# isl-org/Open3D-PointNet2-Semantic3D

Hardware: AMD Instinct MI355X
Metric: points/sec through SA+FP stack (B=16,N=8192) (higher is better)
Workload: dtype f32

## Files before the change

### include/pn2_abi.h

```cpp
#ifndef PN2_ABI_H_
#define PN2_ABI_H_

#include <stddef.h>
#include <stdint.h>

#ifdef __cplusplus
extern "C" {
#endif

#define PN2_ABI_VERSION 2

#define PN2_OK 0
#define PN2_EINVAL (-1)
#define PN2_ENULL (-2)
#define PN2_ERANGE (-3)
#define PN2_EUNSUP (-4)

#define PN2_ARITH_STRICT 0
#define PN2_ARITH_FMA 1
#define PN2_ARITH_FMA_ALT 2

int pn2_abi_version(void);
const char *pn2_build_info(void);
const char *pn2_strerror(int code);
// ... 228 lines not shown
                                  const float *z, int nlayers, const int *widths, const float *const *w,
                                  const float *const *bias, float *y, int schedule, void *stream);

int pn2_set_sa_row_packing(int on);

int pn2_sa_mlp_fused_pre(int b, int n, int m, int nsample, const float *xyz, const float *new_xyz, const float *zf,
                         const int *idx, int nlayers, const int *widths, const float *const *w,
                         const float *const *bias, int pool, float *out, void *stream);

int pn2_fp_mlp_wide_pre(int b, int n, int m, int c1, const float *dist, const int *idx, const float *points1,
                        const float *z, int nlayers, const int *widths, const float *const *w,
                        const float *const *bias, float *y, void *stream);
int pn2_sa_mlp_wide_pre(int b, int n, int m, int nsample, const float *xyz, const float *new_xyz, const float *zf,
                        const int *idx, int nlayers, const int *widths, const float *const *w,
                        const float *const *bias, int pool, float *y, void *stream);

size_t pn2_ball_query_bin_bytes(int n);
int pn2_ball_query_bin(int b, int n, float radius, const float *xyz1, void *workspace, size_t workspace_bytes, void *stream);
int pn2_ball_query_bin_ld(int b, int n, float radius, const float *xyz1, int ld1, void *workspace, size_t workspace_bytes,
                          void *stream);
int pn2_query_ball_point_binned(int b, int n, int m, float radius, int nsample, const float *xyz1, const float *xyz2,
                                const void *bins, int *idx, int *pts_cnt, int arith_mode, void *stream);

int pn2_group_pool(long long rows, int k, int c, int mode, const float *x, const float *gxyz, float *out, void *stream);
int pn2_group_pool_grad(long long rows, int k, int c, int mode, const float *x, const float *gxyz, const float *dout,
                        float *dx, void *stream);

int pn2_bn_relu_forward_deferred(long long rows, int c, const float *y, const float *gamma, const float *beta,
                                 const float *bias, float eps, float decay, int stats_done, float *running_mean,
                                 float *running_var, void *workspace, size_t workspace_bytes, float *save_mean,
// ... 82 lines not shown
```

### open3d-pointnet2-semantic3d_amd/_lib.py

```python
import ctypes
import os
import sys

import torch

_HERE = os.path.dirname(os.path.abspath(__file__))
LIB_PATH = os.environ.get("PN2_HIP_LIBRARY") or os.path.join(_HERE, "libpn2_hip.so")

c_int, c_float, c_void_p = ctypes.c_int, ctypes.c_float, ctypes.c_void_p

SIGNATURES = {
    "pn2_farthest_point_sample": [c_int, c_int, c_int, c_void_p, c_void_p, c_void_p, c_int, c_void_p],
    "pn2_fps_gather": [c_int, c_int, c_int, c_void_p, c_void_p, c_void_p, c_void_p, c_int, c_void_p],
    "pn2_fps_nested": [c_int, c_int, c_int, c_void_p, c_void_p, c_void_p, c_void_p, c_void_p, c_void_p, c_int, c_void_p],
    "pn2_fps_nested_ld": [c_int, c_int, c_int, c_void_p, c_int, c_void_p, c_void_p, c_void_p, c_void_p, c_int, c_void_p],
    "pn2_coarse_geometry": [c_int, c_int, c_int, c_void_p, c_void_p, c_void_p, c_void_p, c_void_p, c_void_p, c_void_p, c_void_p,
                            c_void_p, c_void_p, c_void_p, c_void_p, c_int, c_int, c_void_p],
    "pn2_prob_sample": [c_int, c_int, c_int, c_void_p, c_void_p, c_void_p, c_void_p, c_void_p],
    "pn2_fps_large": [c_int, c_int, c_int, c_void_p, c_void_p, ctypes.c_size_t, c_void_p, c_void_p, c_int, c_void_p],
    "pn2_gather_point": [c_int, c_int, c_int, c_void_p, c_void_p, c_void_p, c_void_p],
    "pn2_gather_point_grad": [c_int, c_int, c_int, c_void_p, c_void_p, c_void_p, c_void_p],
    "pn2_query_ball_point": [c_int, c_int, c_int, c_float, c_int, c_void_p, c_void_p, c_void_p, c_void_p, c_int, c_void_p],
    "pn2_query_ball_point_ld": [c_int, c_int, c_int, c_float, c_int, c_void_p, c_int, c_void_p, c_void_p, c_void_p, c_int, c_void_p],
    "pn2_query_ball_point_kernel": [c_int, c_int, c_int, c_float, c_int, c_void_p, c_void_p, c_void_p, c_void_p, c_int, c_int,
# ... 109 lines not shown
                                c_void_p, c_void_p, c_void_p],
    "pn2_scene_sample": [c_int, c_int, c_int, c_void_p, c_void_p, c_void_p, c_void_p, c_void_p, c_void_p, ctypes.c_double,
                         ctypes.c_double, c_void_p, c_void_p, c_void_p, c_void_p, c_void_p, c_void_p, c_void_p],
    "pn2_fp_mlp_fused_pre": [c_int, c_int, c_int, c_int, c_void_p, c_void_p, c_void_p, c_void_p, c_int, c_void_p, c_void_p,
                             c_void_p, c_void_p, c_void_p],
    "pn2_fp_mlp_fused_pre_ld": [c_int, c_int, c_int, c_int, c_void_p, c_void_p, c_void_p, c_int, c_void_p, c_int, c_void_p, c_void_p,
                                c_void_p, c_void_p, c_void_p],
    "pn2_fp_mlp_fused_pre_schedule": [c_int, c_int, c_int, c_int, c_void_p, c_void_p, c_void_p, c_void_p, c_int, c_void_p,
                                      c_void_p, c_void_p, c_void_p, c_int, c_void_p],
    "pn2_sa_mlp_fused_pre": [c_int, c_int, c_int, c_int, c_void_p, c_void_p, c_void_p, c_void_p, c_int, c_void_p, c_void_p,
                             c_void_p, c_int, c_void_p, c_void_p],
    "pn2_fp_mlp_wide_pre": [c_int, c_int, c_int, c_int, c_void_p, c_void_p, c_void_p, c_void_p, c_int, c_void_p, c_void_p,
                            c_void_p, c_void_p, c_void_p],
    "pn2_sa_mlp_wide_pre": [c_int, c_int, c_int, c_int, c_void_p, c_void_p, c_void_p, c_void_p, c_int, c_void_p, c_void_p,
                            c_void_p, c_int, c_void_p, c_void_p],
    "pn2_ball_query_bin": [c_int, c_int, c_float, c_void_p, c_void_p, ctypes.c_size_t, c_void_p],
    "pn2_ball_query_bin_ld": [c_int, c_int, c_float, c_void_p, c_int, c_void_p, ctypes.c_size_t, c_void_p],
    "pn2_query_ball_point_binned": [c_int, c_int, c_int, c_float, c_int, c_void_p, c_void_p, c_void_p, c_void_p, c_void_p, c_int,
                                    c_void_p],
    "pn2_group_pool": [ctypes.c_longlong, c_int, c_int, c_int, c_void_p, c_void_p, c_void_p, c_void_p],
    "pn2_group_pool_grad": [ctypes.c_longlong, c_int, c_int, c_int, c_void_p, c_void_p, c_void_p, c_void_p, c_void_p],
    "pn2_voxel_downsample": [c_int, c_void_p, c_void_p, c_void_p, ctypes.c_double, c_void_p, c_void_p, c_void_p, c_void_p,
                             c_void_p, c_void_p, ctypes.c_size_t, c_void_p],
    "pn2_dataset_workspace_size": [c_int, c_int, c_void_p],
    "pn2_dataset_sample": [c_int, c_int, c_int, c_int, c_int, c_int, c_void_p, c_void_p, c_void_p, c_void_p, c_void_p, c_void_p,
                           c_void_p, c_int, ctypes.c_double, ctypes.c_double, ctypes.c_ulonglong, c_void_p, c_void_p, c_void_p,
                           c_void_p, c_int, c_void_p, c_void_p, ctypes.c_size_t, c_void_p, c_void_p, c_void_p, c_void_p,
                           c_void_p, c_void_p, c_void_p],
}
PN2_EUNSUP = -4
BN_WS_UNCLEARED, BN_WS_ZEROED, BN_WS_SUMMED, BN_WS_FOLDED = range(4)
_SIZE_QUERIES = {"pn2_fps_large_workspace_bytes": 2, "pn2_ball_query_bin_bytes": 1, "pn2_interpolate_label_workspace_bytes": 1,
                 "pn2_three_interpolate_grad_workspace_bytes": 3, "pn2_scatter_plan_bytes": 3,
                 "pn2_group_point_grad_workspace_bytes": 4, "pn2_voxel_downsample_workspace_bytes": 1, "pn2_bn_workspace_bytes": 1}
_TRACE_ARGS = {"pn2_sa_mlp_max_fused": (9, 10, None, ()), "pn2_sa_mlp_rows_fused": (9, 10, None, ()),
               "pn2_sa_mlp_max_fused_bf16": (9, 10, None, ()), "pn2_fp_mlp_fused": (9, 10, None, ()),
               "pn2_fp_mlp_wide_pre": (8, 9, None, ()), "pn2_sa_mlp_wide_pre": (8, 9, None, ()),
               "pn2_sa_mlp_fused_pre": (8, 9, None, ()), "pn2_fp_mlp_fused_pre": (8, 9, None, ()),
               "pn2_fp_mlp_fused_pre_schedule": (8, 9, None, ()), "pn2_mlp_chain": (3, 4, None, ()),
               "pn2_mlp_wide": (4, 5, None, ()), "pn2_fp_mlp_wide": (9, 10, None, ()), "pn2_sa_mlp_wide": (9, 10, None, ()),
               "pn2_fps_nested_ld": (None, None, "pn2_fps_nested", (3,)),
               "pn2_query_ball_point_ld": (None, None, "pn2_query_ball_point", (5,)),
               "pn2_three_nn_ld": (None, None, "pn2_three_nn", (3,)),
               "pn2_ball_query_bin_ld": (None, None, "pn2_ball_query_bin", (3,)),
               "pn2_sa_mlp_max_fused_ld": (11, 12, "pn2_sa_mlp_max_fused", (5, 6)),
               "pn2_fp_mlp_fused_pre_ld": (9, 10, "pn2_fp_mlp_fused_pre", (4,))}


class Pn2Error(RuntimeError):
    pass


def _load():
    import fcntl
    from . import build as _build
# ... 155 lines not shown
```

### open3d-pointnet2-semantic3d_amd/csrc/pn2_mlp_wide.hip

```cpp
#include "pn2_common.h"

namespace {

typedef float f32x4 __attribute__((ext_vector_type(4)));
typedef float f32x16 __attribute__((ext_vector_type(16)));

constexpr int kWideDepth = 4;

struct WideParams {
    int rows, cin, x_stride, nlayers, pool, relu_last;
    int w[3];
    const float* x;
    int n, m, c;
    const float* xyz;
    const float* new_xyz;
    const float* points;
    const int* idx;
    const float* dist;
    const float* points1;
    int c1, c2;
    const float* W[3];
    const float* bias[3];
    float* y;
    const float* zpre;
// ... 290 lines not shown
                    for (int t = 0; t < 4; ++t) acc[t][r] += z[t];
                }
            } else if constexpr (MODE == kWideGather) {
                const float* __restrict__ zb = p.zpre + (size_t)(tile / p.m) * p.n * N + cb + 4 * l31;
                const int* __restrict__ idx = p.idx + (size_t)tile * 32;
#pragma unroll
                for (int r = 0; r < 16; ++r) {
                    const int row = (r & 3) + 8 * (r >> 2) + 4 * half;
                    const f32x4 z = *reinterpret_cast<const f32x4*>(zb + (size_t)idx[row] * N);
#pragma unroll
                    for (int t = 0; t < 4; ++t) acc[t][r] += z[t];
                }
            }
        }
        if (ks == 0) {
            const f32x4 bv = *reinterpret_cast<const f32x4*>(p.bias[l] + cb + 4 * l31);
            const bool relu = !lastl || p.relu_last;
            if (!lastl) {
                float* __restrict__ out = smem + buf_off[(l + 1) & 1];
                const int so = p.sa[(l + 1) & 1];
#pragma unroll
                for (int r = 0; r < 16; ++r) {
                    const int row = (r & 3) + 8 * (r >> 2) + 4 * half;
                    f32x4 v = {acc[0][r] + bv[0], acc[1][r] + bv[1], acc[2][r] + bv[2], acc[3][r] + bv[3]};
                    v = {fmaxf(v[0], 0.f), fmaxf(v[1], 0.f), fmaxf(v[2], 0.f), fmaxf(v[3], 0.f)};
                    *reinterpret_cast<f32x4*>(out + row * so + cb + 4 * l31) = v;
                }
            } else if (p.pool == 32) {
                f32x4 v;
#pragma unroll
                for (int t = 0; t < 4; ++t) {
// ... 43 lines not shown
            if ((size_t)32 * p.sa[l & 1] < (size_t)2 * 64 * 64) alias_ok = false;
        }
        kin = p.w[l];
    }
    (void)kin;
    p.scratch_off = 32 * (p.sa[0] + p.sa[1]);
    p.scratch_alias = sliced && alias_ok;
    p.rowtab_off = p.scratch_off + (sliced && !alias_ok ? 2 * 64 * 64 : 0);
    const size_t lds = sizeof(float) * ((size_t)p.rowtab_off + (p.zpre && mode == kWideInterp ? 32 * 8 : 0));
    if (lds > kPn2CuLdsBytes) return PN2_EUNSUP;
    if (mode == kWideGather) return launch_mlp_wide_mode<kWideGather>(p, lds, st);
    if (mode == kWideInterp) return launch_mlp_wide_mode<kWideInterp>(p, lds, st);
    return launch_mlp_wide_mode<kWidePlain>(p, lds, st);
}

int check_layers(int nlayers, const int* widths, const float* const* w, const float* const* bias) {
    if (nlayers < 1 || nlayers > 3) return PN2_EUNSUP;
    if (!widths || !w || !bias) return PN2_ENULL;
    for (int l = 0; l < nlayers; ++l) {
        if (widths[l] != 128 && widths[l] != 256 && widths[l] != 512) return PN2_EUNSUP;
        if (!w[l] || !bias[l]) return PN2_ENULL;
        if ((((uintptr_t)w[l]) | ((uintptr_t)bias[l])) & 15) return PN2_EUNSUP;
    }
    return PN2_OK;
}

}

extern "C" int pn2_mlp_wide(int rows, int cin, int x_stride, const float* x, int nlayers, const int* widths,
                            const float* const* w, const float* const* bias, int relu_last, int pool, float* y, void* stream) {
    if (rows <= 0 || cin <= 0 || x_stride < cin) return PN2_EINVAL;
    if (!x || !y) return PN2_ENULL;
    int rc = check_layers(nlayers, widths, w, bias);
    if (rc != PN2_OK) return rc;
    if (pool != 0 && pool != 32) return PN2_EUNSUP;
    if (pool == 32 && rows % 32 != 0) return PN2_EINVAL;
    if (((uintptr_t)y) & 15) return PN2_EUNSUP;
    if ((long long)rows + 64 > 0x7fffffffLL) return PN2_ERANGE;
    WideParams p = {};
    p.rows = rows; p.cin = cin; p.x_stride = x_stride; p.nlayers = nlayers; p.pool = pool; p.relu_last = relu_last;
    p.x = x; p.y = y;
    for (int l = 0; l < nlayers; ++l) { p.w[l] = widths[l]; p.W[l] = w[l]; p.bias[l] = bias[l]; }
    return launch_mlp_wide(p, kWidePlain, static_cast<hipStream_t>(stream));
}

extern "C" int pn2_sa_mlp_wide(int b, int n, int m, int nsample, int c, const float* xyz, const float* new_xyz,
                               const float* points, const int* idx, int nlayers, const int* widths, const float* const* w,
                               const float* const* bias, int pool, float* y, void* stream) {
    if (b <= 0 || n <= 0 || m <= 0 || c <= 0) return PN2_EINVAL;
    if (!xyz || !new_xyz || !points || !idx || !y) return PN2_ENULL;
    if (nsample != 32 || c % 4 != 0 || (((uintptr_t)points | (uintptr_t)y) & 15)) return PN2_EUNSUP;
    int rc = check_layers(nlayers, widths, w, bias);
    if (rc != PN2_OK) return rc;
    if ((long long)b * m * 32 + 64 > 0x7fffffffLL) return PN2_ERANGE;
    WideParams p = {};
    p.rows = b * m * 32; p.cin = 3 + c; p.x_stride = 0; p.nlayers = nlayers; p.pool = pool ? 32 : 0; p.relu_last = 1;
    p.n = n; p.m = m; p.c = c; p.xyz = xyz; p.new_xyz = new_xyz; p.points = points; p.idx = idx; p.y = y;
    for (int l = 0; l < nlayers; ++l) { p.w[l] = widths[l]; p.W[l] = w[l]; p.bias[l] = bias[l]; }
// ... 4 lines not shown
                               const float* points2, int nlayers, const int* widths, const float* const* w,
                               const float* const* bias, float* y, void* stream) {
    if (b <= 0 || n <= 0 || m < 3 || c2 <= 0 || c1 < 0) return PN2_EINVAL;
    if (!dist || !idx || !points2 || !y || (c1 > 0 && !points1)) return PN2_ENULL;
    if (n % 32 != 0 || c2 % 4 != 0 || c1 % 4 != 0 || (((uintptr_t)points2 | (uintptr_t)points1 | (uintptr_t)y) & 15)) return PN2_EUNSUP;
    int rc = check_layers(nlayers, widths, w, bias);
    if (rc != PN2_OK) return rc;
    if ((long long)b * n + 64 > 0x7fffffffLL) return PN2_ERANGE;
    WideParams p = {};
    p.rows = b * n; p.cin = c2 + c1; p.nlayers = nlayers; p.pool = 0; p.relu_last = 1;
    p.n = n; p.m = m; p.c1 = c1; p.c2 = c2; p.dist = dist; p.idx = idx; p.points = points2; p.points1 = points1; p.y = y;
    for (int l = 0; l < nlayers; ++l) { p.w[l] = widths[l]; p.W[l] = w[l]; p.bias[l] = bias[l]; }
    return launch_mlp_wide(p, kWideInterp, static_cast<hipStream_t>(stream));
}

extern "C" int pn2_fp_mlp_wide_pre(int b, int n, int m, int c1, const float* dist, const int* idx, const float* points1,
                                   const float* z, int nlayers, const int* widths, const float* const* w,
                                   const float* const* bias, float* y, void* stream) {
    if (b <= 0 || n <= 0 || m < 3 || c1 <= 0) return PN2_EINVAL;
    if (!dist || !idx || !z || !y || !points1) return PN2_ENULL;
    if (n % 32 != 0 || c1 % 4 != 0 || (((uintptr_t)z | (uintptr_t)points1 | (uintptr_t)y) & 15)) return PN2_EUNSUP;
    int rc = check_layers(nlayers, widths, w, bias);
    if (rc != PN2_OK) return rc;
    if ((long long)b * n + 64 > 0x7fffffffLL) return PN2_ERANGE;
    WideParams p = {};
    p.rows = b * n; p.cin = c1; p.nlayers = nlayers; p.pool = 0; p.relu_last = 1;
    p.n = n; p.m = m; p.c1 = c1; p.c2 = 0; p.dist = dist; p.idx = idx; p.points = nullptr; p.points1 = points1; p.y = y; p.zpre = z;
    for (int l = 0; l < nlayers; ++l) { p.w[l] = widths[l]; p.W[l] = w[l]; p.bias[l] = bias[l]; }
    return launch_mlp_wide(p, kWideInterp, static_cast<hipStream_t>(stream));
}

extern "C" int pn2_sa_mlp_wide_pre(int b, int n, int m, int nsample, const float* xyz, const float* new_xyz, const float* zf,
                                   const int* idx, int nlayers, const int* widths, const float* const* w,
                                   const float* const* bias, int pool, float* y, void* stream) {
    if (b <= 0 || n <= 0 || m <= 0) return PN2_EINVAL;
    if (!xyz || !new_xyz || !zf || !idx || !y) return PN2_ENULL;
    if (nsample != 32 || (((uintptr_t)zf | (uintptr_t)y) & 15)) return PN2_EUNSUP;
    int rc = check_layers(nlayers, widths, w, bias);
    if (rc != PN2_OK) return rc;
    if ((long long)b * m * 32 + 64 > 0x7fffffffLL) return PN2_ERANGE;
    WideParams p = {};
    p.rows = b * m * 32; p.cin = 3; p.x_stride = 0; p.nlayers = nlayers; p.pool = pool ? 32 : 0; p.relu_last = 1;
    p.n = n; p.m = m; p.c = 4; p.xyz = xyz; p.new_xyz = new_xyz; p.points = zf; p.idx = idx; p.y = y; p.zpre = zf;
    for (int l = 0; l < nlayers; ++l) { p.w[l] = widths[l]; p.W[l] = w[l]; p.bias[l] = bias[l]; }
// ... 3 lines not shown
```

### open3d-pointnet2-semantic3d_amd/model.py

```python
import json

import torch

from .util import tf_util
from .util import pointnet_util as pu
from .util.pointnet_util import pointnet_fp_module, pointnet_sa_module
from .tf_ops.tf_interpolate import three_nn

SEMANTIC_HYPERPARAMS = {
    "num_point": 8192, "batch_size": 16, "use_color": 1,
    "optimizer": "adam", "momentum": 0.9, "learning_rate": 0.001, "decay_step": 200000, "learning_rate_decay_rate": 0.7,
    "bn_init_decay": 0.5, "bn_decay_decay_rate": 0.5, "bn_decay_clip": 0.99,
    "l1_radius": 0.5, "l1_nsample": 32, "l1_npoint": 1024,
    "l2_radius": 1.0, "l2_nsample": 32, "l2_npoint": 256,
    "l3_radius": 2.0, "l3_nsample": 32, "l3_npoint": 64,
    "l4_radius": 4.0, "l4_nsample": 32, "l4_npoint": 16,
}

SA_MLPS = ([32, 32, 64], [64, 64, 128], [128, 128, 256], [256, 256, 512])
FP_MLPS = ([256, 256], [256, 256], [256, 128], [128, 128, 128])


def load_hyperparams(path):
    with open(path) as f:
# ... 107 lines not shown
            xyzs[-1], feats[-1], npoint=hyperparams[k + "npoint"], radius=hyperparams[k + "radius"],
            nsample=hyperparams[k + "nsample"], mlp=list(SA_MLPS[li]), mlp2=None, group_all=False,
            is_training=is_training, bn_decay=bn_decay, scope="layer%d" % (li + 1), geometry=geo)
        if li == 0 and geometry is None:
            coarse = coarse_levels(new_xyz, hyperparams)
        xyzs.append(new_xyz)
        feats.append(new_points)

    fp_in = feats
    if cut_sa_fp and is_training:
        fp_in = [feats[0]] + [f.detach().requires_grad_(True) for f in feats[1:]]
        end_points["sa_features_cut"] = fp_in[1:]
    up = fp_in[4]
    for fi in range(4):
        lvl = 3 - fi
        up = pointnet_fp_module(xyzs[lvl], xyzs[lvl + 1], fp_in[lvl], up, list(FP_MLPS[fi]), is_training, bn_decay,
                                scope="fa_layer%d" % (fi + 1),
                                nn=(tuple(geometry["nn"][fi]) + (geometry.get("iplans", [None] * 4)[fi],) if geometry is not None
                                    else (tuple(coarse[2 - fi]["nn"]) + (None,) if (coarse is not None and fi < 3) else None)),
                                defer_last_bn=head_width if (fi == 3 and is_training) else 0)
    end_points["xyzs"] = xyzs
    end_points["sa_features"] = feats
    return up, end_points


def get_head(l0_points, is_training, num_class, bn_decay=None, end_points=None):
    net = tf_util.conv1d(l0_points, 128, 1, padding="VALID", bn=True, is_training=is_training, scope="fc1",
                         bn_decay=bn_decay)
    if end_points is not None:
        end_points["feats"] = net
    net = tf_util.dropout(net, keep_prob=0.5, is_training=is_training, scope="dp1")
    return tf_util.conv1d(net, num_class, 1, padding="VALID", activation_fn=None, scope="fc2", is_training=is_training)


def get_model(point_cloud, is_training, num_class, hyperparams, bn_decay=None, geometry=None, cut_sa_fp=False):
# ... 38 lines not shown
```

### open3d-pointnet2-semantic3d_amd/util/pointnet_util.py

```python

import torch

from . import tf_util
from .._lib import float_array, int_array, launch, lib, ptr, ptr_table, require_cuda, rows_in_place, u64_array
from ..tf_ops import tf_grouping
from ..tf_ops.tf_grouping import query_ball_point_multi, group_point, knn_point, query_ball_point
from ..tf_ops.tf_interpolate import three_interpolate, three_nn
from ..tf_ops.tf_sampling import (farthest_point_sample, farthest_point_sample_and_gather, farthest_point_sample_with_ties,
                                  gather_point, tag_fps_output)


def sample_and_group(npoint, radius, nsample, xyz, points, knn=False, use_xyz=True, geometry=None):
    plan = None
    if geometry is not None:
        new_xyz, idx = geometry[0], geometry[1]
        plan = geometry[2] if len(geometry) > 2 else None
    else:
        fps_idx, fps_tie, _ = farthest_point_sample_with_ties(npoint, xyz)
        new_xyz = tag_fps_output(gather_point(xyz, fps_idx), fps_tie)
        if knn:
            _, idx = knn_point(nsample, xyz, new_xyz)
        else:
            idx, pts_cnt = query_ball_point(radius, nsample, xyz, new_xyz)
    if USE_FUSED_TRAIN_FRONT and points is not None and use_xyz and points.dtype == torch.float32:
# ... 505 lines not shown
    return out


USE_FUSED_TRAIN_FRONT = True


USE_MLP_CHAIN = True


USE_MLP_WIDE = True
WIDE_MIN_ROWS = 4096


USE_FUSED_FP = True


def dense_mlp_inference(x2d, cin, mlp, scope_fmt, bn=True, fp_front=None):
    if x2d is None:
        dist, idx, points1, points2, pad_to = fp_front
        rows = dist.shape[0] * dist.shape[1]
        cw = -(-cin // pad_to) * pad_to
    else:
        rows, cw = x2d.shape
    folded = []
    c = cin
    for i, cout in enumerate(mlp):
        with tf_util.variable_scope(scope_fmt % i):
            pad_in = cw if i == 0 else None
            folded.append(tf_util.folded_dense(c, cout, bn, (1, 1, c, cout), pad_to=32, pad_in=pad_in))
        c = cout
    i, h = 0, x2d
    if h is None:
        if (USE_FUSED_FP and USE_MLP_CHAIN and USE_HOISTED_FP and rows >= 65536 and len(mlp) >= 2
                and all(w <= 128 and w % 32 == 0 for w in mlp[:3])):
            take = min(3, len(mlp))
            y = tf_util.hip_fp_mlp_fused_pre(dist, idx, points1, points2, [folded[k][0] for k in range(take)],
                                             [folded[k][1] for k in range(take)])
            if y is not None:
                h, i = y, take
        if h is None and points1 is not None:
            points1 = points1.contiguous()
        if (h is None and USE_FUSED_FP and USE_MLP_CHAIN and rows >= 65536 and points2.shape[2] % 8 == 0
                and mlp[0] <= 128 and mlp[0] % 32 == 0):
            for take in (2, 1):
                if take > len(mlp) or any(w > 128 or w % 32 for w in mlp[:take]):
                    continue
                y = tf_util.hip_fp_mlp_fused(dist, idx, points1, points2, [folded[k][0] for k in range(take)],
                                             [folded[k][1] for k in range(take)])
                if y is not None:
                    h, i = y, take
                    break
        if (h is None and USE_FUSED_FP and USE_MLP_WIDE and WIDE_MIN_ROWS <= rows <= 65536 and dist.shape[1] % 32 == 0
                and points2.shape[2] % 4 == 0 and (points1 is None or points1.shape[2] % 4 == 0)
                and all(w in (128, 256, 512) for w in mlp[:3])):
            take = min(3, len(mlp))
            y = None
            if USE_HOISTED_FP and points1 is not None:
                y = tf_util.hip_fp_mlp_wide_pre(dist, idx, points1, points2, [folded[k][0] for k in range(take)],
                                                [folded[k][1] for k in range(take)])
            if y is None:
                y = tf_util.hip_fp_mlp_wide(dist, idx, points1, points2, [folded[k][0] for k in range(take)],
                                            [folded[k][1] for k in range(take)])
            if y is not None:
                h, i = y, take
        if h is None:
            x = _fp_interp_concat(dist, idx, points1, points2, pad_to=pad_to)
            h = x.reshape(rows, x.shape[2])
    while i < len(mlp):
        done = False
        if USE_MLP_WIDE and WIDE_MIN_ROWS <= h.shape[0] <= 65536 and all(w in (128, 256, 512) for w in mlp[i:i + 3]):
            take = min(3, len(mlp) - i)
            y = tf_util.hip_mlp_wide(h, [folded[k][0] for k in range(i, i + take)], [folded[k][1] for k in range(i, i + take)])
            if y is not None:
                h, i = y, i + take
                continue
        if USE_MLP_CHAIN and h.shape[0] >= 65536 and all(w <= 128 and w % 32 == 0 for w in mlp[i:i + 2]):
            for take in (2, 1):
                if i + take > len(mlp) or any(w > 128 or w % 32 for w in mlp[i:i + take]):
                    continue
                y = tf_util.hip_mlp_chain(h, [folded[k][0] for k in range(i, i + take)],
                                          [folded[k][1] for k in range(i, i + take)])
                if y is not None:
                    h, i, done = y, i + take, True
                    break
        if not done:
            w2, b2 = folded[i]
            h = tf_util.hip_linear(h, w2, b2, relu=True)
            if h.shape[1] != mlp[i]:
                h = h[:, :mlp[i]].contiguous()
            i += 1
    return h


def fp_features_inference(dist, idx, points1, points2, mlp, bn=True, bn_decay=None):
    b, n = dist.shape[0], dist.shape[1]
    cin = points2.shape[2] + (0 if points1 is None else points1.shape[2])
    h = dense_mlp_inference(None, cin, mlp, "conv_%d", bn, fp_front=(dist, idx, points1, points2, 8))
    return h.reshape(b, n, mlp[-1])


def pointnet_fp_module(xyz1, xyz2, points1, points2, mlp, is_training, bn_decay, scope, bn=True, nn=None, defer_last_bn=0):
    require_cuda(xyz1, xyz2, points1, points2)
    with tf_util.variable_scope(scope):
        dist, idx = (nn[0], nn[1]) if nn is not None else three_nn(xyz1, xyz2)
        plan = nn[2] if nn is not None and len(nn) > 2 else None
        if not is_training:
            return fp_features_inference(dist, idx, points1, points2, mlp, bn, bn_decay)
        c1 = 0 if points1 is None else points1.shape[2]
        if (tf_util.USE_HOISTED_TRAIN and bn and points1 is not None
                and 1 <= c1 <= 8 and not points1.requires_grad
                and points1.dtype == torch.float32 and points2.dtype == torch.float32 and len(mlp) > 0 and mlp[0] % 32 == 0
                and _plan_usable(plan, mlp[0])):
            rows = points1.shape[0] * points1.shape[1]
            nxt = list(mlp[1:]) + [int(defer_last_bn)]
            defer = lambda i: bn and nxt[i] > 0 and tf_util.can_defer_bn(rows, mlp[i], nxt[i])
            h = tf_util.conv2d_hoisted_first("fp", points2, (dist, idx, points1), plan, points2.shape[2] + points1.shape[2],
                                             mlp[0], "conv_0", bn_decay, defer_bn=defer(0))
            for i, cout in enumerate(mlp):
                if i > 0:
                    h = tf_util.conv2d(h, cout, [1, 1], padding="VALID", stride=[1, 1], bn=bn, is_training=is_training,
                                       scope="conv_%d" % i, bn_decay=bn_decay, defer_bn=defer(i))
            return h.squeeze(2)
# ... 18 lines not shown
```

### open3d-pointnet2-semantic3d_amd/util/tf_util.py

```python
import contextlib
import math
from collections import OrderedDict

import weakref

import torch
import torch.nn.functional as F

from .._lib import BN_WS_FOLDED, BN_WS_SUMMED, BN_WS_UNCLEARED, BN_WS_ZEROED
from .._lib import int_array, launch, layer_arrays, lib, nbytes, ptr, ptr_table, require_cuda, rows_in_place, u64_array

BN_EPSILON = 1e-3


class VariableStore:

    def __init__(self, device="cuda", seed=0):
        self.device = torch.device(device)
        self.params = OrderedDict()
        self.buffers = OrderedDict()
        self._gen = torch.Generator(device="cpu")
        self._gen.manual_seed(seed)
        self._seed = int(seed)
        self._dropout = {}
# ... 235 lines not shown


def hip_mlp_wide(x2d, ws, bs, relu_last=True, pool=0):
    require_cuda(x2d)
    x2d = x2d.contiguous()
    rows, cin = x2d.shape
    if ws[0].shape[0] < -(-cin // 8) * 8:
        ws = [F.pad(ws[0], (0, 0, 0, -(-cin // 8) * 8 - ws[0].shape[0])).contiguous()] + list(ws[1:])
    L, widths, wptrs, bptrs = layer_arrays(ws, bs)
    y = torch.empty((rows // pool if pool else rows, ws[-1].shape[1]), dtype=torch.float32, device=x2d.device)
    ok = launch("pn2_mlp_wide", x2d, rows, cin, cin, ptr(x2d), L, widths, wptrs, bptrs, int(bool(relu_last)), int(pool), ptr(y),
                may_refuse=True)
    return y if ok else None


def hip_fp_mlp_wide(dist, idx, points1, points2, ws, bs):
    require_cuda(dist, idx, points1, points2)
    b, n, _ = dist.shape
    m, c2 = points2.shape[1], points2.shape[2]
    c1 = 0 if points1 is None else points1.shape[2]
    need = -(-(c1 + c2) // 8) * 8
    if ws[0].shape[0] < need:
        ws = [F.pad(ws[0], (0, 0, 0, need - ws[0].shape[0])).contiguous()] + list(ws[1:])
    L, widths, wptrs, bptrs = layer_arrays(ws, bs)
    y = torch.empty((b * n, ws[-1].shape[1]), dtype=torch.float32, device=dist.device)
    p1 = None if points1 is None else points1.contiguous()
    ok = launch("pn2_fp_mlp_wide", dist, b, n, m, c1, c2, ptr(dist.contiguous()), ptr(idx.contiguous()), ptr(p1),
                ptr(points2.contiguous()), L, widths, wptrs, bptrs, ptr(y), may_refuse=True)
    return y if ok else None

# ... 5 lines not shown


def hip_sa_mlp_wide(xyz, new_xyz, points, idx, ws, bs, pool=True):
    require_cuda(xyz, new_xyz, points, idx)
    b, n, _ = xyz.shape
    m, ns = idx.shape[1], idx.shape[2]
    c = points.shape[2]
    L, widths, wptrs, bptrs = layer_arrays(ws, bs)
    wl = ws[-1].shape[1]
    y = torch.empty((b, m, wl) if pool else (b, m, ns, wl), dtype=torch.float32, device=xyz.device)
    ok = launch("pn2_sa_mlp_wide", xyz, b, n, m, ns, c, ptr(xyz.contiguous()), ptr(new_xyz.contiguous()), ptr(points.contiguous()),
                ptr(idx.contiguous()), L, widths, wptrs, bptrs, int(bool(pool)), ptr(y), may_refuse=True)
    return y if ok else None


def hip_fp_mlp_wide_pre(dist, idx, points1, points2, ws, bs):
    require_cuda(dist, idx, points1, points2)
    if points1 is None:
        return None
    b, n, _ = dist.shape
    m, c2 = points2.shape[1], points2.shape[2]
    c1 = points1.shape[2]
    w0a, w0b = split_first_layer(ws[0], c2, c1, "fp_wide_pre", pad_b_rows=8)
    z = hoist_gemm(points2.reshape(b * m, c2), w0a)
    L, widths, wptrs, bptrs = layer_arrays([w0b] + list(ws[1:]), bs)
    y = torch.empty((b * n, ws[-1].shape[1]), dtype=torch.float32, device=dist.device)
    ok = launch("pn2_fp_mlp_wide_pre", dist, b, n, m, c1, ptr(dist.contiguous()), ptr(idx.contiguous()), ptr(points1.contiguous()),
                ptr(z), L, widths, wptrs, bptrs, ptr(y), may_refuse=True)
    return y if ok else None


def hip_sa_mlp_wide_pre(xyz, new_xyz, points, idx, ws, bs, pool=True):
    require_cuda(xyz, new_xyz, points, idx)
    b, n, _ = xyz.shape
    m, ns = idx.shape[1], idx.shape[2]
    c = points.shape[2]
    w0f, w0x = split_first_layer(ws[0], c, 3, "sa_wide_pre", pad_b_rows=8)
    zf = hoist_gemm(points.reshape(b * n, c), w0f)
    L, widths, wptrs, bptrs = layer_arrays([w0x] + list(ws[1:]), bs)
    wl = ws[-1].shape[1]
    y = torch.empty((b, m, wl) if pool else (b, m, ns, wl), dtype=torch.float32, device=xyz.device)
    ok = launch("pn2_sa_mlp_wide_pre", xyz, b, n, m, ns, ptr(xyz.contiguous()), ptr(new_xyz.contiguous()), ptr(zf),
                ptr(idx.contiguous()), L, widths, wptrs, bptrs, int(bool(pool)), ptr(y), may_refuse=True)
# ... 2 lines not shown

def hip_fp_mlp_fused(dist, idx, points1, points2, ws, bs):
    require_cuda(dist, idx, points1, points2)
    b, n, _ = dist.shape
    m, c2 = points2.shape[1], points2.shape[2]
    c1 = 0 if points1 is None else points1.shape[2]
    p1 = None if points1 is None else points1.contiguous()
    p2 = points2.contiguous()
    L, widths, wptrs, bptrs = layer_arrays(ws, bs)
    y = torch.empty((b * n, ws[-1].shape[1]), dtype=torch.float32, device=dist.device)
    ok = launch("pn2_fp_mlp_fused", dist, b, n, m, c1, c2, ptr(dist.contiguous()), ptr(idx.contiguous()), ptr(p1), ptr(p2), L, widths,
                wptrs, bptrs, ptr(y), may_refuse=True)
    return y if ok else None


_zero_bias = {}
HOIST_GEMM_WIDE = False


def hoist_gemm(x2d, w):
    rows, cin = x2d.shape
    cout = w.shape[1]
    if HOIST_GEMM_WIDE and 4096 <= rows <= 65536 and cout in (128, 256, 512) and cin % 8 == 0:
        key = (cout, str(w.device))
        zb = _zero_bias.get(key)
        if zb is None:
            zb = _zero_bias[key] = torch.zeros(cout, dtype=torch.float32, device=w.device)
        y = hip_mlp_wide(x2d.contiguous(), [w], [zb], relu_last=False)
        if y is not None:
            return y
    return hip_linear(x2d, w, None, relu=False)


def split_first_layer(w2, c2, c1, key, pad_b_rows=None):
    st = get_default_store()

    def make():
        w1b = w2[c2:c2 + c1] if c1 > 0 else None
        if w1b is not None and pad_b_rows and c1 % pad_b_rows:
            w1b = F.pad(w1b, (0, 0, 0, pad_b_rows - c1 % pad_b_rows))
        return w2[:c2].contiguous(), (None if w1b is None else w1b.contiguous())
    return st.folded((_full_name("split"), key, c2, c1, pad_b_rows), [w2], make)


def hip_fp_mlp_fused_pre(dist, idx, points1, points2, ws, bs, schedule=None):
    require_cuda(dist, idx, points1, points2)
    b, n, _ = dist.shape
    m, c2 = points2.shape[1], points2.shape[2]
    c1 = 0 if points1 is None else points1.shape[2]
    L = len(ws)
    if L < 2 or L > 3 or any(w.shape[1] % 32 or w.shape[1] > 128 for w in ws):
        return None
    w1a, w1b = split_first_layer(ws[0], c2, c1, "fp_pre")
    z = hoist_gemm(points2.reshape(b * m, c2), w1a)
    p1, ld1 = (None, 0) if points1 is None else rows_in_place(points1)
    if schedule is not None and p1 is not None:
        p1, ld1 = p1.contiguous(), c1
    widths, wptrs, bptrs = int_array([w.shape[1] for w in ws]), ptr_table([w1b] + list(ws[1:])), ptr_table(bs)
    y = torch.empty((b * n, ws[-1].shape[1]), dtype=torch.float32, device=dist.device)
    common = (b, n, m, c1, ptr(dist.contiguous()), ptr(idx.contiguous()), ptr(p1), ptr(z), L, widths, wptrs, bptrs, ptr(y))
    if schedule is None and p1 is not None and ld1 != c1:
        ok = launch("pn2_fp_mlp_fused_pre_ld", dist, *common[:7], ld1, *common[7:], may_refuse=True)
    elif schedule is None:
        ok = launch("pn2_fp_mlp_fused_pre", dist, *common, may_refuse=True)
    else:
        ok = launch("pn2_fp_mlp_fused_pre_schedule", dist, *common, int(schedule), may_refuse=True)
    return y if ok else None


def hip_linear_narrow(x2d, w, b=None):
    require_cuda(x2d, w, b)
    rows, cin = x2d.shape
    cout = w.shape[1]
    if cout > 16 or cin % 4 != 0 or x2d.dtype != torch.float32:
        return None
    x2d = x2d.contiguous()
    y = torch.empty((rows, cout), dtype=torch.float32, device=x2d.device)
    ok = launch("pn2_linear_narrow", x2d, rows, cin, cout, ptr(x2d), ptr(w.contiguous()), ptr(None if b is None else b.contiguous()),
                ptr(y), may_refuse=True)
    return y if ok else None

# ... 868 lines not shown
```

Baseline: 370.6 million.

## Fuse next FP level's hoisted first-layer GEMM into producing FP wide MLP kernel

In inference, the FP module now precomputes the next FP level's first-layer projection (points2 @ W0a) inside the producing level's fused wide MLP kernel. It appends the consumer weight as an extra bias-free linear layer and hands the result over as HoistedRows. This removes a separate hoist GEMM launch and a write and re-read of the intermediate features. In exchange it adds a layer to the wide kernel, cross-level coupling, and error paths for when a consumer kernel refuses the hoisted rows.

```diff
diff --git a/include/pn2_abi.h b/include/pn2_abi.h
--- a/include/pn2_abi.h
+++ b/include/pn2_abi.h
@@ -266,6 +266,12 @@
 int pn2_sa_mlp_wide_pre(int b, int n, int m, int nsample, const float *xyz, const float *new_xyz, const float *zf,
                         const int *idx, int nlayers, const int *widths, const float *const *w,
                         const float *const *bias, int pool, float *y, void *stream);
+
+int pn2_mlp_wide_z(int rows, int cin, int x_stride, const float *x, int nlayers, const int *widths,
+                   const float *const *w, const float *const *bias, int pool, float *z, void *stream);
+int pn2_fp_mlp_wide_pre_z(int b, int n, int m, int c1, const float *dist, const int *idx, const float *points1,
+                          const float *z, int nlayers, const int *widths, const float *const *w,
+                          const float *const *bias, float *z_out, void *stream);
 
 size_t pn2_ball_query_bin_bytes(int n);
 int pn2_ball_query_bin(int b, int n, float radius, const float *xyz1, void *workspace, size_t workspace_bytes, void *stream);
diff --git a/open3d-pointnet2-semantic3d_amd/_lib.py b/open3d-pointnet2-semantic3d_amd/_lib.py
--- a/open3d-pointnet2-semantic3d_amd/_lib.py
+++ b/open3d-pointnet2-semantic3d_amd/_lib.py
@@ -147,6 +147,9 @@
                             c_void_p, c_void_p, c_void_p],
     "pn2_sa_mlp_wide_pre": [c_int, c_int, c_int, c_int, c_void_p, c_void_p, c_void_p, c_void_p, c_int, c_void_p, c_void_p,
                             c_void_p, c_int, c_void_p, c_void_p],
+    "pn2_mlp_wide_z": [c_int, c_int, c_int, c_void_p, c_int, c_void_p, c_void_p, c_void_p, c_int, c_void_p, c_void_p],
+    "pn2_fp_mlp_wide_pre_z": [c_int, c_int, c_int, c_int, c_void_p, c_void_p, c_void_p, c_void_p, c_int, c_void_p, c_void_p,
+                              c_void_p, c_void_p, c_void_p],
     "pn2_ball_query_bin": [c_int, c_int, c_float, c_void_p, c_void_p, ctypes.c_size_t, c_void_p],
     "pn2_ball_query_bin_ld": [c_int, c_int, c_float, c_void_p, c_int, c_void_p, ctypes.c_size_t, c_void_p],
     "pn2_query_ball_point_binned": [c_int, c_int, c_int, c_float, c_int, c_void_p, c_void_p, c_void_p, c_void_p, c_void_p, c_int,
@@ -171,7 +174,8 @@
                "pn2_fp_mlp_wide_pre": (8, 9, None, ()), "pn2_sa_mlp_wide_pre": (8, 9, None, ()),
                "pn2_sa_mlp_fused_pre": (8, 9, None, ()), "pn2_fp_mlp_fused_pre": (8, 9, None, ()),
                "pn2_fp_mlp_fused_pre_schedule": (8, 9, None, ()), "pn2_mlp_chain": (3, 4, None, ()),
-               "pn2_mlp_wide": (4, 5, None, ()), "pn2_fp_mlp_wide": (9, 10, None, ()), "pn2_sa_mlp_wide": (9, 10, None, ()),
+               "pn2_mlp_wide": (4, 5, None, ()), "pn2_mlp_wide_z": (4, 5, None, ()), "pn2_fp_mlp_wide_pre_z": (8, 9, None, ()),
+               "pn2_fp_mlp_wide": (9, 10, None, ()), "pn2_sa_mlp_wide": (9, 10, None, ()),
                "pn2_fps_nested_ld": (None, None, "pn2_fps_nested", (3,)),
                "pn2_query_ball_point_ld": (None, None, "pn2_query_ball_point", (5,)),
                "pn2_three_nn_ld": (None, None, "pn2_three_nn", (3,)),
diff --git a/open3d-pointnet2-semantic3d_amd/csrc/pn2_mlp_wide.hip b/open3d-pointnet2-semantic3d_amd/csrc/pn2_mlp_wide.hip
--- a/open3d-pointnet2-semantic3d_amd/csrc/pn2_mlp_wide.hip
+++ b/open3d-pointnet2-semantic3d_amd/csrc/pn2_mlp_wide.hip
@@ -328,7 +328,7 @@
             }
         }
         if (ks == 0) {
-            const f32x4 bv = *reinterpret_cast<const f32x4*>(p.bias[l] + cb + 4 * l31);
+            const f32x4 bv = p.bias[l] ? *reinterpret_cast<const f32x4*>(p.bias[l] + cb + 4 * l31) : f32x4{0.f, 0.f, 0.f, 0.f};
             const bool relu = !lastl || p.relu_last;
             if (!lastl) {
                 float* __restrict__ out = smem + buf_off[(l + 1) & 1];
@@ -402,12 +402,12 @@
     return launch_mlp_wide_mode<kWidePlain>(p, lds, st);
 }
 
-int check_layers(int nlayers, const int* widths, const float* const* w, const float* const* bias) {
+int check_layers(int nlayers, const int* widths, const float* const* w, const float* const* bias, bool plain_last = false) {
     if (nlayers < 1 || nlayers > 3) return PN2_EUNSUP;
     if (!widths || !w || !bias) return PN2_ENULL;
     for (int l = 0; l < nlayers; ++l) {
         if (widths[l] != 128 && widths[l] != 256 && widths[l] != 512) return PN2_EUNSUP;
-        if (!w[l] || !bias[l]) return PN2_ENULL;
+        if (!w[l] || (!bias[l] && !(plain_last && l == nlayers - 1))) return PN2_ENULL;
         if ((((uintptr_t)w[l]) | ((uintptr_t)bias[l])) & 15) return PN2_EUNSUP;
     }
     return PN2_OK;
@@ -415,11 +415,12 @@
 
 }
 
-extern "C" int pn2_mlp_wide(int rows, int cin, int x_stride, const float* x, int nlayers, const int* widths,
-                            const float* const* w, const float* const* bias, int relu_last, int pool, float* y, void* stream) {
+namespace {
+int mlp_wide_entry(int rows, int cin, int x_stride, const float* x, int nlayers, const int* widths, const float* const* w,
+                   const float* const* bias, int relu_last, bool plain_last, int pool, float* y, void* stream) {
     if (rows <= 0 || cin <= 0 || x_stride < cin) return PN2_EINVAL;
     if (!x || !y) return PN2_ENULL;
-    int rc = check_layers(nlayers, widths, w, bias);
+    int rc = check_layers(nlayers, widths, w, bias, plain_last);
     if (rc != PN2_OK) return rc;
     if (pool != 0 && pool != 32) return PN2_EUNSUP;
     if (pool == 32 && rows % 32 != 0) return PN2_EINVAL;
@@ -430,6 +431,17 @@
     p.x = x; p.y = y;
     for (int l = 0; l < nlayers; ++l) { p.w[l] = widths[l]; p.W[l] = w[l]; p.bias[l] = bias[l]; }
     return launch_mlp_wide(p, kWidePlain, static_cast<hipStream_t>(stream));
+}
+}
+
+extern "C" int pn2_mlp_wide(int rows, int cin, int x_stride, const float* x, int nlayers, const int* widths,
+                            const float* const* w, const float* const* bias, int relu_last, int pool, float* y, void* stream) {
+    return mlp_wide_entry(rows, cin, x_stride, x, nlayers, widths, w, bias, relu_last, false, pool, y, stream);
+}
+
+extern "C" int pn2_mlp_wide_z(int rows, int cin, int x_stride, const float* x, int nlayers, const int* widths,
+                              const float* const* w, const float* const* bias, int pool, float* z, void* stream) {
+    return mlp_wide_entry(rows, cin, x_stride, x, nlayers, widths, w, bias, 0, true, pool, z, stream);
 }
 
 extern "C" int pn2_sa_mlp_wide(int b, int n, int m, int nsample, int c, const float* xyz, const float* new_xyz,
@@ -464,20 +476,35 @@
     return launch_mlp_wide(p, kWideInterp, static_cast<hipStream_t>(stream));
 }
 
+namespace {
+int fp_mlp_wide_pre_entry(int b, int n, int m, int c1, const float* dist, const int* idx, const float* points1, const float* z,
+                          int nlayers, const int* widths, const float* const* w, const float* const* bias, bool plain_last,
+                          float* y, void* stream) {
+    if (b <= 0 || n <= 0 || m < 3 || c1 <= 0) return PN2_EINVAL;
+    if (!dist || !idx || !z || !y || !points1) return PN2_ENULL;
+    if (n % 32 != 0 || c1 % 4 != 0 || (((uintptr_t)z | (uintptr_t)points1 | (uintptr_t)y) & 15)) return PN2_EUNSUP;
+    int rc = check_layers(nlayers, widths, w, bias, plain_last);
+    if (rc != PN2_OK) return rc;
+    if ((long long)b * n + 64 > 0x7fffffffLL) return PN2_ERANGE;
+    WideParams p = {};
+    p.rows = b * n; p.cin = c1; p.nlayers = nlayers; p.pool = 0; p.relu_last = plain_last ? 0 : 1;
+    p.n = n; p.m = m; p.c1 = c1; p.c2 = 0; p.dist = dist; p.idx = idx; p.points = nullptr; p.points1 = points1; p.y = y; p.zpre = z;
+    for (int l = 0; l < nlayers; ++l) { p.w[l] = widths[l]; p.W[l] = w[l]; p.bias[l] = bias[l]; }
+    return launch_mlp_wide(p, kWideInterp, static_cast<hipStream_t>(stream));
+}
+}
+
 extern "C" int pn2_fp_mlp_wide_pre(int b, int n, int m, int c1, const float* dist, const int* idx, const float* points1,
                                    const float* z, int nlayers, const int* widths, const float* const* w,
                                    const float* const* bias, float* y, void* stream) {
-    if (b <= 0 || n <= 0 || m < 3 || c1 <= 0) return PN2_EINVAL;
-    if (!dist || !idx || !z || !y || !points1) return PN2_ENULL;
-    if (n % 32 != 0 || c1 % 4 != 0 || (((uintptr_t)z | (uintptr_t)points1 | (uintptr_t)y) & 15)) return PN2_EUNSUP;
-    int rc = check_layers(nlayers, widths, w, bias);
-    if (rc != PN2_OK) return rc;
-    if ((long long)b * n + 64 > 0x7fffffffLL) return PN2_ERANGE;
-    WideParams p = {};
-    p.rows = b * n; p.cin = c1; p.nlayers = nlayers; p.pool = 0; p.relu_last = 1;
-    p.n = n; p.m = m; p.c1 = c1; p.c2 = 0; p.dist = dist; p.idx = idx; p.points = nullptr; p.points1 = points1; p.y = y; p.zpre = z;
-    for (int l = 0; l < nlayers; ++l) { p.w[l] = widths[l]; p.W[l] = w[l]; p.bias[l] = bias[l]; }
-    return launch_mlp_wide(p, kWideInterp, static_cast<hipStream_t>(stream));
+    return fp_mlp_wide_pre_entry(b, n, m, c1, dist, idx, points1, z, nlayers, widths, w, bias, false, y, stream);
+}
+
+extern "C" int pn2_fp_mlp_wide_pre_z(int b, int n, int m, int c1, const float* dist, const int* idx, const float* points1,
+                                     const float* z, int nlayers, const int* widths, const float* const* w,
+                                     const float* const* bias, float* z_out, void* stream) {
+    if (nlayers < 2) return PN2_EUNSUP;
+    return fp_mlp_wide_pre_entry(b, n, m, c1, dist, idx, points1, z, nlayers, widths, w, bias, true, z_out, stream);
 }
 
 extern "C" int pn2_sa_mlp_wide_pre(int b, int n, int m, int nsample, const float* xyz, const float* new_xyz, const float* zf,
diff --git a/open3d-pointnet2-semantic3d_amd/model.py b/open3d-pointnet2-semantic3d_amd/model.py
--- a/open3d-pointnet2-semantic3d_amd/model.py
+++ b/open3d-pointnet2-semantic3d_amd/model.py
@@ -145,11 +145,15 @@
     up = fp_in[4]
     for fi in range(4):
         lvl = 3 - fi
+        consumer = None
+        if fi < 3 and not is_training:
+            consumer = ("fa_layer%d" % (fi + 2), xyzs[lvl - 1].shape[1], 0 if fp_in[lvl - 1] is None else fp_in[lvl - 1].shape[2],
+                        FP_MLPS[fi + 1])
         up = pointnet_fp_module(xyzs[lvl], xyzs[lvl + 1], fp_in[lvl], up, list(FP_MLPS[fi]), is_training, bn_decay,
                                 scope="fa_layer%d" % (fi + 1),
                                 nn=(tuple(geometry["nn"][fi]) + (geometry.get("iplans", [None] * 4)[fi],) if geometry is not None
                                     else (tuple(coarse[2 - fi]["nn"]) + (None,) if (coarse is not None and fi < 3) else None)),
-                                defer_last_bn=head_width if (fi == 3 and is_training) else 0)
+                                defer_last_bn=head_width if (fi == 3 and is_training) else 0, consumer=consumer)
     end_points["xyzs"] = xyzs
     end_points["sa_features"] = feats
     return up, end_points
diff --git a/open3d-pointnet2-semantic3d_amd/util/pointnet_util.py b/open3d-pointnet2-semantic3d_amd/util/pointnet_util.py
--- a/open3d-pointnet2-semantic3d_amd/util/pointnet_util.py
+++ b/open3d-pointnet2-semantic3d_amd/util/pointnet_util.py
@@ -543,12 +543,48 @@
 
 USE_FUSED_FP = True
 
-
-def dense_mlp_inference(x2d, cin, mlp, scope_fmt, bn=True, fp_front=None):
+USE_PRODUCER_HOIST = True
+USE_PRODUCER_HOIST_FP_WIDE = True
+USE_PRODUCER_HOIST_FP_TAIL = False
+
+
+def _fp_hoist_route(rows, n, c2, c1, mlp):
+    if (USE_FUSED_FP and USE_MLP_CHAIN and USE_HOISTED_FP and rows >= 65536 and len(mlp) >= 2
+            and all(w <= 128 and w % 32 == 0 for w in mlp[:3])):
+        return "fp_pre", None
+    if (USE_FUSED_FP and USE_MLP_WIDE and USE_HOISTED_FP and WIDE_MIN_ROWS <= rows <= 65536 and n % 32 == 0 and c2 % 4 == 0
+            and 0 < c1 <= 512 and c1 % 4 == 0 and all(w in (128, 256, 512) for w in mlp[:3])):
+        return "fp_wide_pre", 8
+    return None
+
+
+def fp_consumer_hoist(scope, b, n, c2, c1, mlp, bn=True):
+    if not USE_PRODUCER_HOIST or not mlp or mlp[0] % 32:
+        return None
+    route = _fp_hoist_route(b * n, n, c2, c1, mlp)
+    if route is None:
+        return None
+    cin = c2 + c1
+    with tf_util.variable_scope(scope):
+        with tf_util.variable_scope("conv_0"):
+            if tf_util._full_name("weights") not in tf_util.get_default_store().params:
+                return None
+            w0 = tf_util.folded_dense(cin, mlp[0], bn, (1, 1, cin, mlp[0]), pad_to=32, pad_in=-(-cin // 8) * 8)[0]
+        return tf_util.split_first_layer(w0, c2, c1, route[0], pad_b_rows=route[1])[0], route[0]
+
+
+def dense_mlp_inference(x2d, cin, mlp, scope_fmt, bn=True, fp_front=None, consumer=None):
+    ready = None
     if x2d is None:
         dist, idx, points1, points2, pad_to = fp_front
         rows = dist.shape[0] * dist.shape[1]
         cw = -(-cin // pad_to) * pad_to
+        c2 = points2.c2 if isinstance(points2, tf_util.HoistedRows) else points2.shape[2]
+        if isinstance(points2, tf_util.HoistedRows):
+            ready = points2
+            if _fp_hoist_route(rows, dist.shape[1], ready.c2, 0 if points1 is None else points1.shape[2], mlp) != (
+                    ready.key, 8 if ready.key == "fp_wide_pre" else None):
+                raise ValueError("hoisted rows made for the %r path reach an FP level that does not take it" % ready.key)
     else:
         rows, cw = x2d.shape
     folded = []
@@ -559,6 +595,11 @@
             folded.append(tf_util.folded_dense(c, cout, bn, (1, 1, c, cout), pad_to=32, pad_in=pad_in))
         c = cout
     i, h = 0, x2d
+    wz = None
+    if consumer is not None and consumer[0].shape[0] == mlp[-1] and consumer[0].shape[1] in (128, 256, 512):
+        wz = consumer[0]
+    emitted = lambda z: tf_util.HoistedRows(z.reshape(-1, rows // dist.shape[0], z.shape[1]) if fp_front is not None
+                                            else z, mlp[-1], consumer[1])
     if h is None:
         if (USE_FUSED_FP and USE_MLP_CHAIN and USE_HOISTED_FP and rows >= 65536 and len(mlp) >= 2
                 and all(w <= 128 and w % 32 == 0 for w in mlp[:3])):
@@ -569,7 +610,7 @@
                 h, i = y, take
         if h is None and points1 is not None:
             points1 = points1.contiguous()
-        if (h is None and USE_FUSED_FP and USE_MLP_CHAIN and rows >= 65536 and points2.shape[2] % 8 == 0
+        if (h is None and USE_FUSED_FP and USE_MLP_CHAIN and rows >= 65536 and ready is None and c2 % 8 == 0
                 and mlp[0] <= 128 and mlp[0] % 32 == 0):
             for take in (2, 1):
                 if take > len(mlp) or any(w > 128 or w % 32 for w in mlp[:take]):
@@ -580,11 +621,16 @@
                     h, i = y, take
                     break
         if (h is None and USE_FUSED_FP and USE_MLP_WIDE and WIDE_MIN_ROWS <= rows <= 65536 and dist.shape[1] % 32 == 0
-                and points2.shape[2] % 4 == 0 and (points1 is None or points1.shape[2] % 4 == 0)
+                and c2 % 4 == 0 and (points1 is None or points1.shape[2] % 4 == 0)
                 and all(w in (128, 256, 512) for w in mlp[:3])):
             take = min(3, len(mlp))
             y = None
             if USE_HOISTED_FP and points1 is not None:
+                if wz is not None and USE_PRODUCER_HOIST_FP_WIDE and take == len(mlp) <= 2:
+                    z = tf_util.hip_fp_mlp_wide_pre(dist, idx, points1, points2, [folded[k][0] for k in range(take)],
+                                                    [folded[k][1] for k in range(take)], z_weight=wz)
+                    if z is not None:
+                        return emitted(z)
                 y = tf_util.hip_fp_mlp_wide_pre(dist, idx, points1, points2, [folded[k][0] for k in range(take)],
                                                 [folded[k][1] for k in range(take)])
             if y is None:
@@ -592,6 +638,8 @@
                                             [folded[k][1] for k in range(take)])
             if y is not None:
                 h, i = y, take
+        if h is None and ready is not None:
+            raise ValueError("hoisted rows reach an FP level whose hoisted launch did not take them")
         if h is None:
             x = _fp_interp_concat(dist, idx, points1, points2, pad_to=pad_to)
             h = x.reshape(rows, x.shape[2])
@@ -614,6 +662,11 @@
                     break
         if not done:
             w2, b2 = folded[i]
+            if (wz is not None and USE_PRODUCER_HOIST_FP_TAIL and USE_MLP_WIDE and i == len(mlp) - 1 and mlp[i] in (128, 256, 512)
+                    and h.shape[0] < WIDE_MIN_ROWS):
+                z = tf_util.hip_mlp_wide_z(h, [w2, wz], [b2, None])
+                if z is not None:
+                    return emitted(z)
             h = tf_util.hip_linear(h, w2, b2, relu=True)
             if h.shape[1] != mlp[i]:
                 h = h[:, :mlp[i]].contiguous()
@@ -621,20 +674,29 @@
     return h
 
 
-def fp_features_inference(dist, idx, points1, points2, mlp, bn=True, bn_decay=None):
+def fp_features_inference(dist, idx, points1, points2, mlp, bn=True, bn_decay=None, consumer=None):
     b, n = dist.shape[0], dist.shape[1]
-    cin = points2.shape[2] + (0 if points1 is None else points1.shape[2])
-    h = dense_mlp_inference(None, cin, mlp, "conv_%d", bn, fp_front=(dist, idx, points1, points2, 8))
-    return h.reshape(b, n, mlp[-1])
-
-
-def pointnet_fp_module(xyz1, xyz2, points1, points2, mlp, is_training, bn_decay, scope, bn=True, nn=None, defer_last_bn=0):
-    require_cuda(xyz1, xyz2, points1, points2)
+    c2 = points2.c2 if isinstance(points2, tf_util.HoistedRows) else points2.shape[2]
+    cin = c2 + (0 if points1 is None else points1.shape[2])
+    h = dense_mlp_inference(None, cin, mlp, "conv_%d", bn, fp_front=(dist, idx, points1, points2, 8), consumer=consumer)
+    return h if isinstance(h, tf_util.HoistedRows) else h.reshape(b, n, mlp[-1])
+
+
+def pointnet_fp_module(xyz1, xyz2, points1, points2, mlp, is_training, bn_decay, scope, bn=True, nn=None, defer_last_bn=0,
+                       consumer=None):
+    ready = isinstance(points2, tf_util.HoistedRows)
+    if ready and is_training:
+        raise ValueError("hoisted rows are an inference-only hand-over")
+    require_cuda(xyz1, xyz2, points1, points2.z if ready else points2)
+    cons = None
+    if consumer is not None and not is_training:
+        cscope, cn, cc1, cmlp = consumer
+        cons = fp_consumer_hoist(cscope, xyz1.shape[0], cn, mlp[-1], cc1, list(cmlp), bn)
     with tf_util.variable_scope(scope):
         dist, idx = (nn[0], nn[1]) if nn is not None else three_nn(xyz1, xyz2)
         plan = nn[2] if nn is not None and len(nn) > 2 else None
         if not is_training:
-            return fp_features_inference(dist, idx, points1, points2, mlp, bn, bn_decay)
+            return fp_features_inference(dist, idx, points1, points2, mlp, bn, bn_decay, consumer=cons)
         c1 = 0 if points1 is None else points1.shape[2]
         if (tf_util.USE_HOISTED_TRAIN and bn and points1 is not None
                 and 1 <= c1 <= 8 and not points1.requires_grad
diff --git a/open3d-pointnet2-semantic3d_amd/util/tf_util.py b/open3d-pointnet2-semantic3d_amd/util/tf_util.py
--- a/open3d-pointnet2-semantic3d_amd/util/tf_util.py
+++ b/open3d-pointnet2-semantic3d_amd/util/tf_util.py
@@ -7,7 +7,7 @@
 import torch
 import torch.nn.functional as F
 
-from .._lib import BN_WS_FOLDED, BN_WS_SUMMED, BN_WS_UNCLEARED, BN_WS_ZEROED
+from .._lib import BN_WS_FOLDED, BN_WS_SUMMED, BN_WS_UNCLEARED, BN_WS_ZEROED, Pn2Error
 from .._lib import int_array, launch, layer_arrays, lib, nbytes, ptr, ptr_table, require_cuda, rows_in_place, u64_array
 
 BN_EPSILON = 1e-3
@@ -273,6 +273,32 @@
     return y if ok else None
 
 
+def hip_mlp_wide_z(x2d, ws, bs, pool=0):
+    require_cuda(x2d)
+    x2d = x2d.contiguous()
+    rows, cin = x2d.shape
+    if ws[0].shape[0] < -(-cin // 8) * 8:
+        ws = [F.pad(ws[0], (0, 0, 0, -(-cin // 8) * 8 - ws[0].shape[0])).contiguous()] + list(ws[1:])
+    L, widths, wptrs, bptrs = layer_arrays(ws, bs)
+    z = torch.empty((rows // pool if pool else rows, ws[-1].shape[1]), dtype=torch.float32, device=x2d.device)
+    ok = launch("pn2_mlp_wide_z", x2d, rows, cin, cin, ptr(x2d), L, widths, wptrs, bptrs, int(pool), ptr(z), may_refuse=True)
+    return z if ok else None
+
+
+class HoistedRows:
+
+    def __init__(self, z, c2, key):
+        self.z, self.c2, self.key = z, int(c2), key
+
+
+def _hoisted_source(points2, b, key):
+    if isinstance(points2, HoistedRows):
+        if points2.key != key or points2.z.shape[0] != b:
+            raise ValueError("hoisted rows made for %r handed to %r" % (points2.key, key))
+        return points2.z.shape[1], points2.c2, points2.z.reshape(b * points2.z.shape[1], points2.z.shape[2])
+    return points2.shape[1], points2.shape[2], None
+
+
 def hip_fp_mlp_wide(dist, idx, points1, points2, ws, bs):
     require_cuda(dist, idx, points1, points2)
     b, n, _ = dist.shape
@@ -308,19 +334,27 @@
     return y if ok else None
 
 
-def hip_fp_mlp_wide_pre(dist, idx, points1, points2, ws, bs):
-    require_cuda(dist, idx, points1, points2)
+def hip_fp_mlp_wide_pre(dist, idx, points1, points2, ws, bs, z_weight=None):
+    require_cuda(dist, idx, points1)
     if points1 is None:
         return None
     b, n, _ = dist.shape
-    m, c2 = points2.shape[1], points2.shape[2]
     c1 = points1.shape[2]
+    m, c2, z = _hoisted_source(points2, b, "fp_wide_pre")
     w0a, w0b = split_first_layer(ws[0], c2, c1, "fp_wide_pre", pad_b_rows=8)
-    z = hoist_gemm(points2.reshape(b * m, c2), w0a)
-    L, widths, wptrs, bptrs = layer_arrays([w0b] + list(ws[1:]), bs)
-    y = torch.empty((b * n, ws[-1].shape[1]), dtype=torch.float32, device=dist.device)
-    ok = launch("pn2_fp_mlp_wide_pre", dist, b, n, m, c1, ptr(dist.contiguous()), ptr(idx.contiguous()), ptr(points1.contiguous()),
+    ready = z is not None
+    if not ready:
+        require_cuda(points2)
+        z = hoist_gemm(points2.reshape(b * m, c2), w0a)
+    lw, lb, name = [w0b] + list(ws[1:]), list(bs), "pn2_fp_mlp_wide_pre"
+    if z_weight is not None:
+        lw, lb, name = lw + [z_weight], lb + [None], name + "_z"
+    L, widths, wptrs, bptrs = layer_arrays(lw, lb)
+    y = torch.empty((b * n, lw[-1].shape[1]), dtype=torch.float32, device=dist.device)
+    ok = launch(name, dist, b, n, m, c1, ptr(dist.contiguous()), ptr(idx.contiguous()), ptr(points1.contiguous()),
                 ptr(z), L, widths, wptrs, bptrs, ptr(y), may_refuse=True)
+    if not ok and ready:
+        raise Pn2Error("%s refused rows whose hoisted product a producing launch has already made" % name)
     return y if ok else None
 
 
@@ -353,7 +387,6 @@
     return y if ok else None
 
 
-_zero_bias = {}
 HOIST_GEMM_WIDE = False
 
 
@@ -361,11 +394,7 @@
     rows, cin = x2d.shape
     cout = w.shape[1]
     if HOIST_GEMM_WIDE and 4096 <= rows <= 65536 and cout in (128, 256, 512) and cin % 8 == 0:
-        key = (cout, str(w.device))
-        zb = _zero_bias.get(key)
-        if zb is None:
-            zb = _zero_bias[key] = torch.zeros(cout, dtype=torch.float32, device=w.device)
-        y = hip_mlp_wide(x2d.contiguous(), [w], [zb], relu_last=False)
+        y = hip_mlp_wide_z(x2d.contiguous(), [w], [None])
         if y is not None:
             return y
     return hip_linear(x2d, w, None, relu=False)
@@ -383,15 +412,20 @@
 
 
 def hip_fp_mlp_fused_pre(dist, idx, points1, points2, ws, bs, schedule=None):
-    require_cuda(dist, idx, points1, points2)
+    require_cuda(dist, idx, points1)
     b, n, _ = dist.shape
-    m, c2 = points2.shape[1], points2.shape[2]
+    m, c2, z = _hoisted_source(points2, b, "fp_pre")
     c1 = 0 if points1 is None else points1.shape[2]
     L = len(ws)
+    ready = z is not None
     if L < 2 or L > 3 or any(w.shape[1] % 32 or w.shape[1] > 128 for w in ws):
+        if ready:
+            raise Pn2Error("pn2_fp_mlp_fused_pre cannot take rows whose hoisted product a producing launch has already made")
         return None
     w1a, w1b = split_first_layer(ws[0], c2, c1, "fp_pre")
-    z = hoist_gemm(points2.reshape(b * m, c2), w1a)
+    if not ready:
+        require_cuda(points2)
+        z = hoist_gemm(points2.reshape(b * m, c2), w1a)
     p1, ld1 = (None, 0) if points1 is None else rows_in_place(points1)
     if schedule is not None and p1 is not None:
         p1, ld1 = p1.contiguous(), c1
@@ -404,6 +438,8 @@
         ok = launch("pn2_fp_mlp_fused_pre", dist, *common, may_refuse=True)
     else:
         ok = launch("pn2_fp_mlp_fused_pre_schedule", dist, *common, int(schedule), may_refuse=True)
+    if not ok and ready:
+        raise Pn2Error("pn2_fp_mlp_fused_pre refused rows whose hoisted product a producing launch has already made")
     return y if ok else None
 
 
```

After: 373.7 million (median of 6 runs). About the same (+0.8%).
